# jmschrei/PyPore

Measured on AMD Instinct MI355X. Metric: Msamples/sec segmented (SpeedyStatSplit, 10^8-sample trace); %HBM roofline, higher is better.
Workload: dtype int32/f64 (exact integer block sums of fp32 or int16 samples; decisions in fp64)

## Files before the change

pypore_amd/csrc/poreseg.hip:

```cpp
#include <hip/hip_runtime.h>

#include <algorithm>
#include <atomic>
#include <chrono>
#include <complex>
#include <cmath>
#include <cstdarg>
#include <cstdio>
#include <cstdlib>
#include <cstring>
#include <initializer_list>
#include <condition_variable>
#include <mutex>
#include <string>
#include <thread>
#include <tuple>
#include <type_traits>
#include <vector>

#include "poreseg.h"
#include "seg_device.hpp"
#include "seg_align.hpp"
#include "seg_pairwise.hpp"
#include "seg_trf.hpp"
// ... 42 lines not shown
struct HostBuf : NoCopy {
    void *p = nullptr;
    size_t cap = 0;
    ~HostBuf() { release(); }
    hipError_t reserve(size_t bytes)
    {
        if (bytes <= cap) return hipSuccess;
        release();
        size_t want = std::max(bytes, cap + cap / 2);
        hipError_t e = hipHostMalloc(&p, want, hipHostMallocDefault);
        if (e == hipSuccess) { cap = want; g_live_bytes += cap; }
        return e;
    }
    void release() { if (p) { (void)hipHostFree(p); g_live_bytes -= cap; } p = nullptr; cap = 0; }
    template <class T> T *as() { return static_cast<T *>(p); }
};

struct Event : NoCopy {
    hipEvent_t e = nullptr;
    ~Event() { if (e) (void)hipEventDestroy(e); }
    operator hipEvent_t() const { return e; }
};

struct Stream : NoCopy {
    hipStream_t s = nullptr;
    bool own = false;
    ~Stream() { if (own && s) (void)hipStreamDestroy(s); }
    operator hipStream_t() const { return s; }
};

}

enum : int { SC_NO_LA = 1, SC_NO_UPLOAD = 2, SC_ALL = 3 };
constexpr int LA_KEEP = 16;
struct ps_ctx {
    int device = 0;
    int n_cu = 0;
    Stream stream;
    Event ev[10];
    Event ev_front[2];
    ~ps_ctx() { (void)hipSetDevice(device); if (stream.s) (void)hipStreamSynchronize(stream.s); }
    std::string err;
    int64_t tile_len = 0, halo = 0;
    int mode = MODE_FAST, spine_nt = 512, tree_nt = 256;
    int lds_max_samples = 0;
    int rep_eval = 1, rep_stage = 1, rep_sum = 1;
    uint8_t *d_is_spine = nullptr;
    int prune = 1;
    double wide_quantum = 0;
    int wide_skip = 0;
    int wide_mode = 0;
    int tree_mw = 0;
    int upload_by_kernel = 1;
    int k0_waves = 0;
    float noise_k = 0.1f;
    int k0_admit = 0;
    int k0_sets = 2;
    bool chain_held = false;
    unsigned long long chain_ticket = 0;
    bool defer_sync = false;
    int scan_lds_pad = 0;
    int k0_unaligned = 1;
    int single_pass = 1;
    int gather_fused = 1;
    int download_by_kernel = 1;
    int debug = 0;
// ... 37 lines not shown
    } trf;
    DevBuf ev_info_tr;
    DevBuf blk_cls, cls_mm;
    DevBuf pre_c;
    struct { DevBuf tab, pre, tmp, stack, cnt, off; } ss;
    struct { DevBuf tab, tab2, mask, cnt, excl, off1, off2, hits, pair_off, keep, kept, y, len, span_off; } sp;
    struct {
        DevBuf log;
        int64_t cap = 65536, hdr_cap = -1;
        int64_t seen = -1, call_cap = 0;
        std::vector<int64_t> ev_start, ev_len;
    } nt;
    struct {
        DevBuf model, off, bp, last, flags;
        std::vector<char> blob;
        long long bp_budget = 512ll << 20;
        DevBuf fmat, acc, skip;
        DevBuf pmax;
        DevBuf samp;
        long long fb_budget = 4ll << 30;
        bool expect_lds = true;
    } hmm;
    int stitch_host = 0;
    DevBuf ev_len, det_counts, det_tics, det_cand;
    DevBuf bridges, bmeta, tile_i32, sp_off, spine_items, asm_hdr, ev_first_tile;
    DevBuf bridge_ext, ext_slot, ext_list;
    DevBuf lat_state, lat_seam, lat_res;
    unsigned lat_tag_next = 1;
    unsigned lat_tag_base = 0;
    int lat_help = 1;
    int bridge_budget = BR_MAX;
    int bridge_ext_on = 1;
    int short_chain = SC_ALL;
    int shared_n = 0;
    int hw_queues = 0;
    int pool_patience = BR_PATIENCE_POOL;
    int la_keep = 0;
    bool la_now = false;
    bool small_clean = false;
    bool small_clean_in = false;
    HostBuf h_hdr;
    DevBuf spine_jobs, spine_scratch, spine_dense, spine_meta, tree_jobs, tree_scratch, tree_spill, tree_defer, screen_acc,
        tree_counts, items, item_pos, first_item, ev_off, bounds_off, small;
    HostBuf h_meta, h_dense, h_small, h_up;
    int timing = 1;
    double ms[8] = {0, 0, 0, 0, 0, 0, 0, 0};
    int64_t counters[20] = {0, 0, 0, 0, 0, 0, 0, 0, 0, 0, 0, 0, 0, 0, -1, -1, 0, 0, 0, 0};
    bool screen_ran = false;
};

namespace {

int fail(ps_ctx *ctx, int code, const char *fmt, ...)
{
    if (ctx) {
        char buf[512];
        va_list ap;
        va_start(ap, fmt);
        vsnprintf(buf, sizeof buf, fmt, ap);
        va_end(ap);
        ctx->err = buf;
    }
    return code;
}

#define HIP_TRY(ctx, expr)                                                                        \
// ... 73 lines not shown
    }
    c.left[t % K0Chain::RING] = t + 1;
    c.open_max = std::max(c.open_max, ++c.open);
    return PS_OK;
}
int chain_publish(ps_ctx *ctx, int device, hipStream_t st, unsigned long long ticket)
{
    K0Chain &c = g_chain[device & 15];
    std::lock_guard<std::mutex> lk(c.mu);
    const hipError_t e = hipEventRecord(c.ev[ticket % K0Chain::RING], st);
    c.close(ticket, e == hipSuccess);
    if (e != hipSuccess) return fail(ctx, PS_ERR_HIP, "hipEventRecord (K0 gate) failed: %s", hipGetErrorString(e));
    return PS_OK;
}
void chain_drop(ps_ctx *ctx)
{
    if (!ctx->chain_held) return;
    ctx->chain_held = false;
    K0Chain &c = g_chain[ctx->device & 15];
    std::lock_guard<std::mutex> lk(c.mu);
    c.close(ctx->chain_ticket, false);
}
constexpr size_t SMALL_TAIL = 64 * 1024;
struct SmallLayout { unsigned long long status, work0, work1, work2, dense, stamp[12], life[9], qctl, qhead, tree_tail; AsmHeader hdr;
                     unsigned long long lat_ctl[6]; int lat_prog[LAT_D];
                     unsigned long long nt_cur;
                     unsigned long long tree_defer[3]; };

int make_cfg(ps_ctx *ctx, const void *d_samples, const ps_sample_format *fmt, int mw, int maxw, int W,
             double min_gain, DevCfg *c)
{
    ctx->small_clean_in = ctx->small_clean;
    ctx->small_clean = false;
    if (!fmt) return fail(ctx, PS_ERR_ARG, "sample format is NULL");
    if (fmt->dtype != PS_DTYPE_F32 && fmt->dtype != PS_DTYPE_I16)
        return fail(ctx, PS_ERR_ARG, "unknown dtype %d", fmt->dtype);
    if (!(fmt->quantum > 0) || !std::isfinite(fmt->quantum))
        return fail(ctx, PS_ERR_ARG, "quantum must be positive and finite");
    c->samples = d_samples;
    c->dtype = fmt->dtype;
    c->off_counts = fmt->dtype == PS_DTYPE_F32 ? 0 : fmt->offset_counts;
    c->dc_counts = fmt->dtype == PS_DTYPE_F32 ? static_cast<double>(fmt->offset_counts) : 0.0;
    c->noise_k = ctx->noise_k;
    c->inv_q = static_cast<float>(1.0 / fmt->quantum);
    c->q = fmt->quantum;
    c->q2 = fmt->quantum * fmt->quantum;
    c->mw = mw; c->maxw = maxw; c->W = W; c->half = W / 2;
    c->min_gain = min_gain;
    c->mode = ctx->mode;
    c->prune = ctx->prune;
    c->lds_cap = std::max(1, std::min(W, ctx->lds_max_samples));
    c->bsum = nullptr; c->ev_info = nullptr; c->chunk_tot = nullptr; c->blk_mm = nullptr; c->grp = nullptr; c->bs_wide = 0;
    c->blk_cls = nullptr; c->cls_mm = nullptr; c->cls_kthr = 0;
    c->k0_unaligned = ctx->k0_unaligned;
    c->pre_c = nullptr; c->pre_c2 = nullptr;
    c->dbg = ctx->small.as<SmallLayout>()->stamp;
    c->nt_log = nullptr;
    c->rep_eval = ctx->rep_eval; c->rep_stage = ctx->rep_stage; c->rep_sum = ctx->rep_sum;
    return PS_OK;
}

inline size_t lds_bytes_for(int lds_cap, int nt)
{
    return (((static_cast<size_t>(lds_cap) + 32) * sizeof(lds_t) + 15) & ~static_cast<size_t>(15)) +
           (static_cast<size_t>(lds_cap) / PBLK + static_cast<size_t>(nt) + 8) * sizeof(int2);
}
// ... 243 lines not shown

inline int64_t spine_cap(int64_t start, int64_t stop, int mw) { return (stop - start) / mw + 4; }

struct TilePlace { int64_t first_tile = 0, ntiles = 1, tile_len = 0x7fffffff, vbase = 0; };
SpineJob make_spine_job(int64_t base, int32_t ev, int64_t len, int64_t start, int64_t stop, int mw, int64_t out_off,
                        const TilePlace &place = TilePlace())
{
    SpineJob j;
    j.base = base;
    j.start = static_cast<int32_t>(start);
    j.end = static_cast<int32_t>(len);
    j.stop = static_cast<int32_t>(stop);
    j.out_cap = static_cast<int32_t>(std::min<int64_t>(spine_cap(start, stop, mw), 0x7fffffff));
    j.out_off = out_off;
    j.first_tile = static_cast<int32_t>(place.first_tile);
    j.ntiles = static_cast<int32_t>(place.ntiles);
    j.tile_len = static_cast<int32_t>(place.tile_len);
    j.ev = ev;
    j.vbase = place.vbase;
    return j;
}

int find_in(const TileList &t, int32_t pos)
{
    if (pos == t.start) return -1;
    auto it = std::lower_bound(t.a.begin(), t.a.end(), pos, [](const Anchor &x, int32_t v) { return x.pos < v; });
    if (it != t.a.end() && it->pos == pos) return static_cast<int>(it - t.a.begin());
    return -2;
}

}

namespace {
constexpr int RC_FALLBACK = 1;
constexpr int RC_WIDE = 2;
int finish_batch(ps_ctx *ctx, const DevCfg &cfg, size_t n_tj, int64_t n_items, int32_t n_ev,
                        int32_t *d_bounds, int64_t cap, int64_t *h_bounds_off, ps_segstat *d_stats,
                        std::chrono::steady_clock::time_point t_begin, const AsmHeader *d_hdr = nullptr,
                        AsmHeader *hdr_out = nullptr, bool wide_check = false)
{
    int rc;
    const size_t evb = (static_cast<size_t>(n_ev) + 1) * sizeof(int64_t);
    SmallLayout *sm = ctx->small.as<SmallLayout>();
    if (ctx->timing >= 2) HIP_TRY(ctx, hipEventRecord(ctx->ev[2], ctx->stream));
    if (n_tj) {
        const unsigned g = static_cast<unsigned>(std::min<size_t>(n_tj, 0x7fffffff));
        if (int lrc = launch_subtrees(ctx, cfg, g, sm, n_tj, d_hdr)) return lrc;
    }
    if (ctx->timing >= 2) HIP_TRY(ctx, hipEventRecord(ctx->ev[3], ctx->stream));
    const bool fused = d_hdr != nullptr && ctx->gather_fused;
    const bool one_copy = ctx->bounds_off.p == ctx->small.as<char>() + sizeof(SmallLayout);
    int dl_clear = 0;
    if (fused) {
        const int64_t blocks = (n_items >> GS_LOG) + 1;
        const unsigned gg = static_cast<unsigned>(std::max<int64_t>(1, std::min<int64_t>(blocks, 1024)));
        hipLaunchKernelGGL(gather_scan_kernel, dim3(gg), dim3(1 << GS_LOG), 0, ctx->stream, ctx->items.as<Item>(),
                           ctx->tree_jobs.as<TreeJob>(), ctx->tree_counts.as<int32_t>(), ctx->tree_scratch.as<int32_t>(),
                           static_cast<long long>(n_items), d_bounds, cap, ctx->d_is_spine, d_hdr, ctx->first_item.as<int64_t>(),
                           n_ev, ctx->bounds_off.as<int64_t>());
        HIP_TRY(ctx, hipGetLastError());
    } else {
    hipLaunchKernelGGL(item_scan_kernel, dim3(1), dim3(1024), 0, ctx->stream, ctx->items.as<Item>(),
                       ctx->tree_counts.as<int32_t>(), n_items, ctx->item_pos.as<int64_t>(), d_hdr,
                       ctx->first_item.as<int64_t>(), n_ev, ctx->bounds_off.as<int64_t>());
    HIP_TRY(ctx, hipGetLastError());
    }
    if (n_items && !fused) {
        const unsigned gg = static_cast<unsigned>(d_hdr ? std::min<int64_t>(n_items, 16384) : n_items);
        hipLaunchKernelGGL(gather_kernel, dim3(gg), dim3(64), 0, ctx->stream,
                           ctx->items.as<Item>(), ctx->tree_jobs.as<TreeJob>(), ctx->tree_counts.as<int32_t>(),
                           ctx->tree_scratch.as<int32_t>(), ctx->item_pos.as<int64_t>(), n_items, d_bounds, cap, ctx->d_is_spine,
                           d_hdr);
        HIP_TRY(ctx, hipGetLastError());
    }
    const bool stats_from_digest = d_stats != nullptr && cfg.bsum != nullptr && cfg.blk_mm != nullptr;
    if (stats_from_digest) {
        const int64_t scap = cap + n_ev;
        const unsigned sg = static_cast<unsigned>(std::min<int64_t>(std::max<int64_t>(scap, 1), 8192));
        by_dtype(cfg.dtype, [&](auto dt) {
            hipLaunchKernelGGL(segstat_bs_kernel<dt()>, dim3(sg), dim3(64), 0, ctx->stream, cfg, ctx->ev_off.as<int64_t>(),
                               ctx->ev_len.as<int64_t>(), n_ev, d_bounds, ctx->bounds_off.as<int64_t>(), d_stats, scap,
                               reinterpret_cast<unsigned *>(&sm->status), d_hdr);
        });
        HIP_TRY(ctx, hipGetLastError());
        if (ctx->timing >= 2) HIP_TRY(ctx, hipEventRecord(ctx->ev[4], ctx->stream));
    }
    if (one_copy) {
        HIP_TRY(ctx, ctx->h_small.reserve(sizeof(SmallLayout) + evb));
// ... 446 lines not shown
#ifdef PS_DIAG
    if (ctx->dbg_phase == 2) {
        if (front) front_lock.unlock();
        HIP_TRY(ctx, hipStreamSynchronize(fs));
        for (int e = 0; e <= n_ev; ++e) h_bounds_off[e] = 0;
        return PS_OK;
    }
#endif
    if (front) {
        HIP_TRY(ctx, hipEventRecord(ctx->ev_front[1], fs));
        front_lock.unlock();
        HIP_TRY(ctx, hipStreamWaitEvent(ctx->stream, ctx->ev_front[1], 0));
    }
    if (nj) {
        const unsigned g = static_cast<unsigned>(nj);
        int lrc;
        if (wide) lrc = launch_scans_bs<DT_WIDE>(ctx, cfg, g, sm);
        else if (use_bs) lrc = launch_scans_bs<0>(ctx, cfg, g, sm);
        else {
            lrc = launch_spine_nt(ctx, cfg, g, sm, true);
            if (lrc) return lrc;
            if (ctx->timing >= 2) HIP_TRY(ctx, hipEventRecord(ctx->ev[6], ctx->stream));
            lrc = by_nt<256, 512>(ctx->spine_nt, [&](auto nt) {
                return by_dtype(cfg.dtype, [&](auto dt) { return launch_bridge<decltype(nt)::value, dt()>(ctx, cfg, g, sm); });
            });
        }
        if (lrc) return lrc;
    }
    if (ctx->timing >= 2) HIP_TRY(ctx, hipEventRecord(ctx->ev[1], ctx->stream));
    int *ti = ctx->tile_i32.as<int>();
    const size_t njp = std::max<size_t>(1, nj);
    const size_t tile_lds = (nj + 1) * sizeof(long long) + 4 * nj * sizeof(int);
    const int use_lds = tile_lds <= 150 * 1024;
    if (use_lds)
        HIP_TRY(ctx, set_dyn_lds(ctx, reinterpret_cast<const void *>(assemble_tiles_kernel), static_cast<int>(tile_lds)));
    AsmHeader hd = {};
    int rc = PS_OK;
    int64_t items_cap = max_items;
    int slots_used = 0, ext_stride = EXT_MAX;
    const bool no_la = nj && no_look_ahead(ctx, cfg);
    bool la_done = false, stride_set = false;
    for (int round = 0;; ++round) {
        hipLaunchKernelGGL(assemble_tiles_kernel, dim3(1), dim3(1024), use_lds ? tile_lds : 0, ctx->stream,
                           static_cast<int>(nj), ctx->spine_meta.as<int4>(), ctx->bmeta.as<int4>(),
                           ctx->ev_first_tile.as<int64_t>(), n_ev, ti, ti + njp, ti + 2 * njp, ti + 3 * njp,
                           ctx->sp_off.as<long long>(), ctx->first_item.as<int64_t>(), ctx->asm_hdr.as<AsmHeader>(),
                           static_cast<long long>(items_cap), use_lds, reinterpret_cast<const unsigned *>(&sm->status));
        HIP_TRY(ctx, hipGetLastError());
        const AsmHeader *d_hdr = ctx->asm_hdr.as<AsmHeader>();
        if (items_cap > 0) {
            const unsigned ag = static_cast<unsigned>(std::min<int64_t>((items_cap + 255) / 256, 2048));
            hipLaunchKernelGGL(assemble_items_kernel, dim3(ag), dim3(256), 0,
                               ctx->stream, ctx->spine_jobs.as<SpineJob>(), static_cast<int>(nj), ctx->spine_meta.as<int4>(),
                               ctx->spine_scratch.as<int2>(), ctx->bridges.as<int2>(), ti + 3 * njp,
                               ctx->sp_off.as<long long>(), static_cast<long long>(items_cap), mw, W, ctx->tree_jobs.as<TreeJob>(),
                               ctx->items.as<Item>(), ctx->tree_counts.as<int32_t>(), d_hdr, cfg.bsum != nullptr ? cfg.ev_info : nullptr,
                               ctx->bridge_ext.as<int2>(), ctx->ext_slot.as<int>(), ext_stride);
            HIP_TRY(ctx, hipGetLastError());
        }
        if (ctx->timing >= 2 && round == 0) HIP_TRY(ctx, hipEventRecord(ctx->ev[5], ctx->stream));
        rc = finish_batch(ctx, cfg, static_cast<size_t>(items_cap), items_cap, n_ev, d_bounds, cap, h_bounds_off, d_stats, t_begin,
                          d_hdr, &hd, use_bs);
        if (rc != RC_FALLBACK || !use_bs || !nj || round == EXT_ROUNDS + (la_done ? 1 : 0) || !ctx->bridge_ext_on) break;
        HIP_TRY(ctx, ctx->h_meta.reserve(2 * nj * sizeof(int4)));
        int4 *h_bm = ctx->h_meta.as<int4>(), *h_mt = h_bm + nj;
        HIP_TRY(ctx, hipMemcpyAsync(h_bm, ctx->bmeta.p, nj * sizeof(int4), hipMemcpyDeviceToHost, ctx->stream));
        HIP_TRY(ctx, hipMemcpyAsync(h_mt, ctx->spine_meta.p, nj * sizeof(int4), hipMemcpyDeviceToHost, ctx->stream));
        HIP_TRY(ctx, hipStreamSynchronize(ctx->stream));
        if (no_la && !la_done) {
            int64_t n_def = 0;
            for (size_t g = 0; g < nj; ++g) n_def += h_bm[g].w == BR_DEFER || h_bm[g].w == BR_DEFER_REACHED;
            if (n_def) {
                if (ctx->debug) fprintf(stderr, "[poreseg] look-ahead kernel behind the stitch: %lld deferred seams\n", static_cast<long long>(n_def));
                HIP_TRY(ctx, hipMemsetAsync(&sm->hdr, 0, sizeof(AsmHeader), ctx->stream));
                if (ctx->tree_screen) HIP_TRY(ctx, hipMemsetAsync(&sm->tree_defer[0], 0, sizeof sm->tree_defer[0], ctx->stream));
                if (int lrc = by_dtype(cfg.dtype, [&](auto dt) { return launch_bridge_la<dt()>(ctx, cfg, static_cast<unsigned>(nj), sm); })) return lrc;
                la_done = true;
                ctx->la_keep = LA_KEEP;
                ctx->counters[4] += n_def;
                ctx->counters[18] += n_def;
                continue;
            }
        }
        std::vector<int> list;
        bool hopeless = false;
        if (!stride_set) {
            size_t n_fail = 0;
            for (size_t g = 0; g < nj; ++g) n_fail += h_bm[g].w == BR_FAIL_REACHED || (h_bm[g].w == BR_FAIL && h_bm[g].x == ctx->bridge_budget);
            ext_stride = n_fail <= static_cast<size_t>(EXT_SLOTS) ? EXT_MAX : EXT_MAX_MANY;
            stride_set = true;
        }
        const int slot_cap = EXT_SLOTS * (EXT_MAX / ext_stride);
        for (size_t g = 0; g < nj; ++g) {
            const bool reached = h_bm[g].w == BR_FAIL_REACHED;
            const bool gave_up = h_bm[g].x == ctx->bridge_budget;
// ... 3 lines not shown
            if (slots_used + static_cast<int>(list.size()) < slot_cap) list.push_back(static_cast<int>(g));
            else if (reached) hopeless = true;
        }
        if (list.empty() || hopeless) break;
        if (ctx->debug) fprintf(stderr, "[poreseg] second chance, round %d: %zu seams continued on the device\n", round + 1, list.size());
        const size_t n_ext = list.size();
        HIP_TRY(ctx, ctx->bridge_ext.reserve(static_cast<size_t>(EXT_SLOTS) * EXT_MAX * sizeof(int2)));
        HIP_TRY(ctx, ctx->ext_slot.reserve(nj * sizeof(int)));
        HIP_TRY(ctx, ctx->ext_list.reserve(static_cast<size_t>(EXT_SLOTS) * (EXT_MAX / EXT_MAX_MANY) * sizeof(int)));
        HIP_TRY(ctx, hipMemcpyAsync(ctx->ext_list.p, list.data(), n_ext * sizeof(int), hipMemcpyHostToDevice, ctx->stream));
        HIP_TRY(ctx, hipStreamSynchronize(ctx->stream));
        HIP_TRY(ctx, hipMemsetAsync(&sm->hdr, 0, sizeof(AsmHeader), ctx->stream));
        if (ctx->tree_screen) HIP_TRY(ctx, hipMemsetAsync(&sm->tree_defer[0], 0, sizeof sm->tree_defer[0], ctx->stream));
        {
            const unsigned g = static_cast<unsigned>(n_ext);
            auto extend = [&](auto dt) {
                hipLaunchKernelGGL((bridge_la_kernel<dt(), true>), dim3(g), dim3(64 * BR_LA), 0, ctx->stream, cfg,
                                   ctx->spine_jobs.as<SpineJob>(), ctx->spine_scratch.as<int2>(), ctx->spine_meta.as<int4>(),
                                   ctx->bridges.as<int2>(), ctx->bmeta.as<int4>(), reinterpret_cast<unsigned *>(&sm->status),
                                   &sm->work0, static_cast<int>(n_ext), ctx->ext_list.as<int>(), ctx->bridge_ext.as<int2>(),
                                   ctx->ext_slot.as<int>(), slots_used, BR_MAX, ext_stride);
            };
            if (wide) by_dtype<DT_WIDE>(cfg.dtype, extend);
            else by_dtype(cfg.dtype, extend);
            HIP_TRY(ctx, hipGetLastError());
        }
        ctx->counters[4] += static_cast<int64_t>(n_ext);
        slots_used += static_cast<int>(n_ext);
        items_cap += static_cast<int64_t>(n_ext) * ext_stride;
        if (int irc = reserve_items(ctx, items_cap, total_len, mw)) return irc;
    }
    ctx->counters[3] = hd.n_items;
    if (slots_used > 0 || la_done) ctx->small_clean = false;
    float ms = 0;
    if (ctx->timing >= 2 && nj && hipEventElapsedTime(&ms, ctx->ev[7], ctx->ev[0]) == hipSuccess) ctx->ms[6] = ms;
    if (ctx->timing >= 2 && nj && hipEventElapsedTime(&ms, ctx->ev[0], ctx->ev[6]) == hipSuccess) ctx->ms[0] = ms;
    if (ctx->timing >= 2 && nj && hipEventElapsedTime(&ms, ctx->ev[6], ctx->ev[1]) == hipSuccess) ctx->ms[5] = ms;
    if (ctx->timing >= 2 && hipEventElapsedTime(&ms, ctx->ev[1], ctx->ev[5]) == hipSuccess) ctx->ms[4] = ms;
    return rc;
}
int device_stitch_batch(ps_ctx *ctx, const DevCfg &cfg_in, int bs_mode, const int64_t *ev_start, const int64_t *ev_len, int32_t n_ev, int mw, int W,
                        int32_t *d_bounds, int64_t cap, int64_t *h_bounds_off, ps_segstat *d_stats,
                        std::chrono::steady_clock::time_point t_begin, bool digest_ready = false)
{
    const int rc = device_stitch_batch_(ctx, cfg_in, bs_mode, ev_start, ev_len, n_ev, mw, W, d_bounds, cap, h_bounds_off, d_stats, t_begin, digest_ready);
    chain_drop(ctx);
    return rc;
}
}

namespace {
std::mutex g_probe_mu;
int g_unaligned_ok[16] = {-1, -1, -1, -1, -1, -1, -1, -1, -1, -1, -1, -1, -1, -1, -1, -1};
int k0_unaligned_probe(int device, hipStream_t st)
{
    std::lock_guard<std::mutex> lk(g_probe_mu);
    int &ok = g_unaligned_ok[device & 15];
    if (ok >= 0) return ok;
    ok = 0;
    unsigned char h[128];
    for (int i = 0; i < 128; ++i) h[i] = static_cast<unsigned char>(37 * i + 11);
    DevBuf d_buf, bad_buf;
    if (d_buf.reserve(256) != hipSuccess || bad_buf.reserve(sizeof(unsigned)) != hipSuccess) { (void)hipGetLastError(); return ok; }
    unsigned char *d = d_buf.as<unsigned char>();
    unsigned *bad = bad_buf.as<unsigned>();
    unsigned hb = 1;
// ... 157 lines not shown
    else if (n == "groups") ctx->groups = value != 0;
    else if (n == "tree_par") ctx->tree_par = value != 0;
    else if (n == "k0_waves" && value >= 0 && value <= 16) ctx->k0_waves = static_cast<int>(value);
    else if (n == "k0_shared") ctx->k0_shared = value != 0;
    else if (n == "k0_admit" && value >= 0) ctx->k0_admit = static_cast<int>(value);
    else if (n == "bridge_ext" && (value == 0 || value == 1)) ctx->bridge_ext_on = static_cast<int>(value);
    else if (n == "lat_help" && value >= 0 && value <= 2) ctx->lat_help = static_cast<int>(value);
    else if (n == "shared_device" && value >= 0 && value <= 4096) {
        ps_pool_plan_t plan;
        if (pool_plan(static_cast<int>(value), ctx->hw_queues > 0 ? ctx->hw_queues : process_hw_queues(), &plan) != PS_OK)
            return fail(ctx, PS_ERR_ARG, "shared_device: no plan for %lld contexts", static_cast<long long>(value));
        ctx->shared_n = static_cast<int>(value);
        ctx->la_keep = 0;
        ctx->k0_waves = plan.k0_waves;
        ctx->lat_help = plan.lat_help;
        ctx->k0_admit = plan.k0_admit;
    }
    else if (n == "hw_queues" && value >= 0 && value <= HW_QUEUES_MAX) ctx->hw_queues = static_cast<int>(value);
    else if (n == "hmm_bp_budget" && value >= 1) ctx->hmm.bp_budget = value;
    else if (n == "hmm_fb_budget" && value >= 1) ctx->hmm.fb_budget = value;
    else if (n == "pairwise_budget" && value >= 1) ctx->pw.budget = value;
    else if (n == "trf_budget" && value >= 1) ctx->trf.budget = value;
    else if (n == "hmm_expect_lds") ctx->hmm.expect_lds = value != 0;
    else if (n == "single_pass") ctx->single_pass = value != 0;
    else if (n == "gather_fused") ctx->gather_fused = value != 0;
    else if (n == "download_by_kernel") ctx->download_by_kernel = value != 0;
    else if (n == "debug") ctx->debug = value != 0;
    else if (n == "k0_unaligned") ctx->k0_unaligned = value != 0 ? k0_unaligned_probe(ctx->device, ctx->stream) : 0;
    else if (n == "slots_pct" && value >= 1 && value <= 100) ctx->slots_pct = static_cast<int>(value);
    else if (n == "tree_jobs_per_wave" && value >= 0 && value <= 1024) ctx->tree_jobs_per_wave = static_cast<int>(value);
    else if (n == "tree_screen") ctx->tree_screen = value != 0;
    else if (n == "short_chain" && value >= 0 && value <= 3) {
        static const int bits[4] = {0, SC_ALL, SC_NO_LA, SC_NO_UPLOAD};
        if (ctx->short_chain != bits[value]) ctx->small_clean = false;
        ctx->short_chain = bits[value];
    }
    else if (n == "bridge_patience" && value >= 1 && value <= 4096) { ctx->pool_patience = static_cast<int>(value); ctx->la_keep = 0; }
    else if (n == "noise_k_ppm" && value >= 0) ctx->noise_k = static_cast<float>(static_cast<double>(value) * 1.0e-6);
#ifdef PS_DIAG
    else if (n == "dbg_phase" && value >= 0 && value <= 2) ctx->dbg_phase = static_cast<int>(value);
    else if (n == "dbg_k0_nogrp") ctx->dbg_k0_nogrp = value != 0;
    else if (n == "cu_mask" && ctx->stream.own)
        return diag_mask_stream(ctx, &ctx->stream.s, static_cast<int>(value & 0xfff), static_cast<int>((value >> 12) & 0xfff),
                                static_cast<int>((value >> 24) & 0xff), ((value >> 32) & 1) != 0);
    else if (n == "k0_sets" && value >= 2 && value <= 4) ctx->k0_sets = static_cast<int>(value);
    else if (n == "scan_lds_pad" && value >= 0 && value <= 65536) ctx->scan_lds_pad = static_cast<int>(value);
    else if (n == "rep_eval" && value >= 1) ctx->rep_eval = static_cast<int>(value);
    else if (n == "rep_stage" && value >= 1) ctx->rep_stage = static_cast<int>(value);
    else if (n == "rep_sum" && value >= 1) ctx->rep_sum = static_cast<int>(value);
#endif
    else if (n == "bridge_budget" && value >= 1 && value <= BR_MAX) ctx->bridge_budget = static_cast<int>(value);
    else if (n == "wide_bs") { ctx->wide_bs = value != 0; ctx->wide_skip = 0; }
    else if (n == "bridge_single" && value >= 1) ctx->bridge_single = static_cast<int>(value);
    else if (n == "tree_tail_pct" && value >= 0 && value <= 100) ctx->tree_tail_pct = static_cast<int>(value);
    else if (n == "filter_fused") ctx->filt.fused = value != 0;
    else if (n == "upload_by_kernel") ctx->upload_by_kernel = value != 0;
    else if (n == "timing") ctx->timing = static_cast<int>(std::max<int64_t>(0, std::min<int64_t>(2, value)));
    else if (n == "tree_mw") ctx->tree_mw = value != 0;
    else if (n == "spine_nt" && (value == 256 || value == 512 || value == 1024)) ctx->spine_nt = static_cast<int>(value);
    else if (n == "tree_nt" && (value == 256 || value == 512)) ctx->tree_nt = static_cast<int>(value);
    else return fail(ctx, PS_ERR_ARG, "unknown option or value: %s", name);
    return PS_OK;
}

int ps_get_option(const ps_ctx *ctx, const char *name, int64_t *value)
{
    if (!ctx || !name || !value) return PS_ERR_ARG;
    const std::string n(name);
    if (n == "k0_waves") *value = ctx->k0_waves;
    else if (n == "k0_admit") *value = ctx->k0_admit;
    else if (n == "lat_help") *value = ctx->lat_help;
    else if (n == "shared_device") *value = ctx->shared_n;
    else if (n == "hw_queues") *value = ctx->hw_queues;
    else return PS_ERR_ARG;
    return PS_OK;
}

int ps_pool_plan(int32_t n_contexts, int32_t hw_queues, ps_pool_plan_t *out) { return pool_plan(n_contexts, hw_queues, out); }

int ps_hw_queues(void) { return process_hw_queues(); }

int ps_gate_stats(int device, int64_t *out, int32_t n_out, int reset)
{
    if (device < 0 || device >= 16 || (!out && n_out > 0) || n_out < 0) return PS_ERR_ARG;
    K0Chain &c = g_chain[device];
    std::lock_guard<std::mutex> lk(c.mu);
    const int64_t v[5] = {static_cast<int64_t>(c.next), c.open, c.open_max, c.host_waits, c.gave_up};
    for (int i = 0; i < n_out; ++i) out[i] = i < 5 ? v[i] : 0;
    if (reset) { c.open_max = c.open; c.host_waits = 0; c.gave_up = 0; }
    return PS_OK;
}

int ps_synchronize(ps_ctx *ctx)
{
    if (!ctx) return PS_ERR_ARG;
    HIP_TRY(ctx, hipStreamSynchronize(ctx->stream));
    return PS_OK;
}

int ps_min_gain(const ps_split_params *p, double *out)
{
    if (!p || !out) return PS_ERR_ARG;
    double fpr = p->false_positive_rate, sps = p->prior_segments_per_second;
    const double sf = p->sampling_freq;
    if (!(fpr != 0.0)) fpr = sf;
    if (!(sps != 0.0)) sps = sf / 2.;
// ... 2207 lines not shown
```

pypore_amd/csrc/seg_device.hpp:

```cpp
#pragma once
#include <hip/hip_runtime.h>
#include <stdint.h>
#include "poreseg.h"

namespace ps {

constexpr int LDS_STACK = 128;
constexpr int MAX_WAVES = 16;
constexpr int OBUF = 256;
constexpr int BR_MAX = 256;
constexpr int LST_MAX = 256;
constexpr int LAT_D = 256;
constexpr int LAT_W = 16;
constexpr int LAT_C = 2048;
constexpr int LAT_TAGS = 4096;
struct LatHelp {
    unsigned long long *ctl;
    unsigned long long *state;
    int *seam;
    int *prog;
    unsigned long long *res;
    unsigned tag_base;
    int stay;
};
// ... 2084 lines not shown
            if (b.w == BR_DEFER) bmeta[g].w = BR_DEFER_REACHED;
        }
    }
    __syncthreads();
    for (int g0 = 0; g0 < n_tiles; g0 += 1024) {
        const int g = g0 + tid;
        long long n = 0;
        if (g < n_tiles && reach[g]) {
            const int c = meta[g].x - entry[g];
            n = static_cast<long long>(c) + bmeta[g].x;
            if (c < 0) fail_s = 1;
        }
        long long e1, e2;
        chunk_exscan2(n, 0, e1, e2, wsum, carry);
        if (g < n_tiles) sp_off[g] = e1;
    }
    const long long n_items = carry[0];
    if (tid == 0) sp_off[n_tiles] = n_items;
    __syncthreads();
    for (int e = tid; e <= n_ev; e += 1024) first_item[e] = sp_off[ev_first_tile[e]];
    if (use_lds)
        for (int g = tid; g <= n_tiles; g += 1024) {
            sp_off_out[g] = sp_off[g];
            if (g < n_tiles) entry_out[g] = entry[g];
        }
    if (tid == 0) {
        hdr->n_items = n_items;
        hdr->n_jobs = n_items;
        hdr->tscratch = 0;
        hdr->fail = (fail_s || n_items > max_items) ? 1 : 0;
    }
}

__global__ __launch_bounds__(256) void assemble_items_kernel(
    const SpineJob *jobs, int n_tiles, const int4 *meta, const int2 *lists, const int2 *bridges,
    const int *entry, const long long *sp_off, long long n_items_host, int mw, int W,
    TreeJob *tjobs, Item *items, int32_t *counts, const AsmHeader *hdr, const int4 *ev_info,
    const int2 *ext = nullptr, const int *ext_slot = nullptr, int ext_stride = EXT_MAX)
{
    const long long n_items = dev_count(hdr, n_items_host);
    for (long long b = blockIdx.x * 256LL + threadIdx.x; b <= (n_items >> GS_LOG); b += gridDim.x * 256LL) counts[n_items_host + b] = 0;
    for (long long i = blockIdx.x * 256LL + threadIdx.x; i < n_items; i += gridDim.x * 256LL) {
    int lo = 0, hi = n_tiles - 1;
    while (lo < hi) {
        const int mid = (lo + hi) >> 1;
        if (sp_off[mid + 1] > i) hi = mid; else lo = mid + 1;
    }
    const int g = lo;
    const int k = static_cast<int>(i - sp_off[g]);
    const int en = entry[g], cnt = meta[g].x;
    const SpineJob jb2 = jobs[g];
    int2 el;
    int pred;
    if (k < cnt - en) {
        el = lists[jb2.out_off + en + k];
        pred = (en + k) > 0 ? lists[jb2.out_off + en + k - 1].x : jb2.start;
    } else {
        const int kb = k - (cnt - en);
        el = bridge_at(bridges, ext, ext_slot, ext_stride, g, kb);
        pred = kb > 0 ? bridge_at(bridges, ext, ext_slot, ext_stride, g, kb - 1).x : (cnt > 0 ? lists[jb2.out_off + cnt - 1].x : jb2.start);
    }
    const bool has = el.y == KIND_HIT || el.y == KIND_LATE;
    Item it;
    it.anchor = el.x;
    it.job = has ? static_cast<int32_t>(i) : -1;
    items[i] = it;
// ... 330 lines not shown
```

pypore_amd/engine.py:

```python
import collections
import ctypes
import os
import threading
import warnings

import numpy as np
import torch

from . import _lib

_contexts = {}

DEFAULT_OPTIONS = {}
DEFAULT_TILING = [0, 0]
POOL_OVERRIDES = {}

EVENT_CAP = 1 << 16

_ENV_OPTIONS = {
    "PORESEG_MODE": "mode", "PORESEG_SPINE_NT": "spine_nt", "PORESEG_TREE_NT": "tree_nt", "PORESEG_PRUNE": "prune",
    "PORESEG_SCAN_BS": "scan_bs", "PORESEG_GROUPS": "groups", "PORESEG_TREE_PAR": "tree_par", "PORESEG_K0_WAVES": "k0_waves",
    "PORESEG_K0_SHARED": "k0_shared", "PORESEG_K0_MAX": "k0_admit", "PORESEG_K0_SETS": "k0_sets", "PORESEG_WIDE_BS": "wide_bs",
    "PORESEG_BRIDGE_SINGLE": "bridge_single", "PORESEG_TREE_TAIL": "tree_tail_pct", "PORESEG_FILTER_FUSED": "filter_fused",
    "PORESEG_UPLOAD": "upload_by_kernel", "PORESEG_TIMING": "timing", "PORESEG_TREE_MW": "tree_mw",
    "PORESEG_TREE_JPW": "tree_jobs_per_wave", "PORESEG_TREE_SCREEN": "tree_screen", "PORESEG_SLOTS_PCT": "slots_pct", "PORESEG_BRIDGE_EXT": "bridge_ext",
    "PORESEG_LAT_HELP": "lat_help", "PORESEG_BRIDGE_BUDGET": "bridge_budget", "PORESEG_DEBUG": "debug",
    "PORESEG_SHORT_CHAIN": "short_chain", "PORESEG_BRIDGE_PATIENCE": "bridge_patience",
    "PORESEG_GATHER_FUSED": "gather_fused", "PORESEG_SINGLE_PASS": "single_pass", "PORESEG_DOWNLOAD": "download_by_kernel", "PORESEG_K0_UNALIGNED": "k0_unaligned",
    "PORESEG_DBG_PHASE": "dbg_phase", "PORESEG_DBG_K0_NOGRP": "dbg_k0_nogrp", "PORESEG_SCAN_LDS_PAD": "scan_lds_pad", "PORESEG_REP_STAGE": "rep_stage",
}


def options_from_env(environ=None):
    env = os.environ if environ is None else environ
    opts = {}
    for var, name in _ENV_OPTIONS.items():
        if var in env and env[var] != "":
            opts[name] = int(env[var])
    if env.get("PORESEG_STITCH"):
        opts["stitch_host"] = 1 if env["PORESEG_STITCH"] == "host" else 0
    if "PORESEG_NOISE_K" in env:
        opts["noise_k_ppm"] = int(round(float(env["PORESEG_NOISE_K"]) * 1e6))
    tiling = [int(env.get("PORESEG_TILE", "0") or 0), int(env.get("PORESEG_HALO", "0") or 0)]
    pool = {}
    if "PORESEG_POOL_K0_WAVES" in env:
        pool["k0_waves"] = int(env["PORESEG_POOL_K0_WAVES"])
    if "PORESEG_POOL_K0_MAX" in env:
        pool["k0_admit"] = int(env["PORESEG_POOL_K0_MAX"])
    if env.get("PORESEG_POOL_SHARED", "0") == "1":
        pool["k0_shared"] = 1
    return opts, tiling, pool


def apply_env_defaults(environ=None):
    opts, tiling, pool = options_from_env(environ)
    DEFAULT_OPTIONS.update(opts)
    if tiling[0] or tiling[1]:
        DEFAULT_TILING[:] = tiling
    POOL_OVERRIDES.update(pool)
    return opts, tiling, pool
# ... 57 lines not shown
            pass

    def set_tiling(self, tile_len=0, halo=0):
        with self.lock:
            _lib.check(self.L.ps_set_tiling(self.handle, int(tile_len), int(halo)), self.handle)

    def set_option(self, name, value):
        with self.lock:
            _lib.check(self.L.ps_set_option(self.handle, name.encode(), int(value)), self.handle)

    def get_option(self, name):
        out = ctypes.c_int64()
        self.L.ps_get_option.argtypes = [ctypes.c_void_p, ctypes.c_char_p, ctypes.POINTER(ctypes.c_int64)]
        with self.lock:
            _lib.check(self.L.ps_get_option(self.handle, name.encode(), ctypes.byref(out)), self.handle)
        return int(out.value)

    def seq_ms(self):
        if not hasattr(self, "_tm"):
            self._tm = ((ctypes.c_double * 8)(), (ctypes.c_int64 * 8)())
        self.L.ps_get_timings(self.handle, self._tm[0], 8, self._tm[1], 8)
        return self._tm[0][7]

    def timings(self):
        ms = (ctypes.c_double * 8)()
        cnt = (ctypes.c_int64 * 20)()
        _lib.check(self.L.ps_get_timings(self.handle, ms, 8, cnt, 20))
        return dict(spine_ms=ms[0], tree_ms=ms[1], gather_ms=ms[2], total_ms=ms[3], stitch_ms=ms[4], bridge_ms=ms[5], blocksum_ms=ms[6], seq_ms=ms[7],
                    windows=cnt[0], candidates=cnt[1], tiles=cnt[2], tree_jobs=cnt[3], repairs=cnt[4],
                    exact_rescans=cnt[5], full_exact_scans=cnt[6], wide_redo=cnt[7],
                    windows_spine=cnt[8], windows_bridge=cnt[9], windows_tree=cnt[10], near_ties=cnt[11],
                    helper_chunks_published=cnt[12], helper_chunks_taken=cnt[13],
                    tree_deferred=cnt[14], windows_screen=cnt[15],
                    lookahead_skipped=cnt[16], upload_skipped=cnt[17], seams_resumed=cnt[18])

    def near_ties(self):
        if not hasattr(self, "_cnt"):
            self._cnt = self.L.ps_counters(self.handle)
        return int(self._cnt[11])

    def near_tie_sites(self):
        with self.lock:
            n = ctypes.c_int64()
            cap = 64
            while True:
                buf = (_lib.NearTie * cap)()
                rc = self.L.ps_get_near_ties(self.handle, buf, cap, ctypes.byref(n))
                if rc == _lib.PS_ERR_CAPACITY and n.value > cap:
                    cap = int(n.value)
                    continue
                _lib.check(rc, self.handle)
                break
            if n.value < 0:
                return None
            return np.frombuffer(buf, dtype=NEAR_TIE_DTYPE, count=int(n.value)).copy()

    @_serialised
    def segment_batch(self, samples, ev_off, params, quantum, offset_counts=0, want_stats=True, cap=None,
                      want_spine=False, lead=0, out=None, near_tie_warning=True):
        assert samples.is_cuda and samples.is_contiguous() and samples.dim() == 1
        if samples.dtype == torch.float32:
            dtype = _lib.PS_DTYPE_F32
        elif samples.dtype == torch.int16:
            dtype = _lib.PS_DTYPE_I16
        else:
            raise ValueError("samples must be float32 or int16, got %s" % samples.dtype)
        ev_off = np.ascontiguousarray(ev_off, dtype=np.int64)
# ... 952 lines not shown
```

Measured before the change: 604,400.

## Add lean single-block tile assembly and size item grids from previous call

```diff
diff --git a/pypore_amd/csrc/poreseg.hip b/pypore_amd/csrc/poreseg.hip
--- a/pypore_amd/csrc/poreseg.hip
+++ b/pypore_amd/csrc/poreseg.hip
@@ -98,6 +98,7 @@
 }
 
 enum : int { SC_NO_LA = 1, SC_NO_UPLOAD = 2, SC_ALL = 3 };
+enum : int { LL_TILES = 1, LL_GRIDS = 2, LL_ALL = 3 };
 constexpr int LA_KEEP = 16;
 struct ps_ctx {
     int device = 0;
@@ -201,6 +202,9 @@
     int bridge_budget = BR_MAX;
     int bridge_ext_on = 1;
     int short_chain = SC_ALL;
+    int lean_launch = LL_ALL;
+    int64_t prev_items = -1;
+    int64_t prev_items_in = -1;
     int shared_n = 0;
     int hw_queues = 0;
     int pool_patience = BR_PATIENCE_POOL;
@@ -340,6 +344,8 @@
 {
     ctx->small_clean_in = ctx->small_clean;
     ctx->small_clean = false;
+    ctx->prev_items_in = ctx->prev_items;
+    ctx->prev_items = -1;
     if (!fmt) return fail(ctx, PS_ERR_ARG, "sample format is NULL");
     if (fmt->dtype != PS_DTYPE_F32 && fmt->dtype != PS_DTYPE_I16)
         return fail(ctx, PS_ERR_ARG, "unknown dtype %d", fmt->dtype);
@@ -649,12 +655,16 @@
 }
 
 namespace {
+unsigned lean_grid(int64_t items)
+{
+    return static_cast<unsigned>(std::min<int64_t>(std::max<int64_t>(64, (2 * items + 255) / 256 + 1), 0x7fffffff));
+}
 constexpr int RC_FALLBACK = 1;
 constexpr int RC_WIDE = 2;
 int finish_batch(ps_ctx *ctx, const DevCfg &cfg, size_t n_tj, int64_t n_items, int32_t n_ev,
                         int32_t *d_bounds, int64_t cap, int64_t *h_bounds_off, ps_segstat *d_stats,
                         std::chrono::steady_clock::time_point t_begin, const AsmHeader *d_hdr = nullptr,
-                        AsmHeader *hdr_out = nullptr, bool wide_check = false)
+                        AsmHeader *hdr_out = nullptr, bool wide_check = false, int64_t lean_items = -1)
 {
     int rc;
     const size_t evb = (static_cast<size_t>(n_ev) + 1) * sizeof(int64_t);
@@ -670,7 +680,8 @@
     int dl_clear = 0;
     if (fused) {
         const int64_t blocks = (n_items >> GS_LOG) + 1;
-        const unsigned gg = static_cast<unsigned>(std::max<int64_t>(1, std::min<int64_t>(blocks, 1024)));
+        unsigned gg = static_cast<unsigned>(std::max<int64_t>(1, std::min<int64_t>(blocks, 1024)));
+        if (lean_items >= 0) gg = std::min(gg, lean_grid(lean_items));
         hipLaunchKernelGGL(gather_scan_kernel, dim3(gg), dim3(1 << GS_LOG), 0, ctx->stream, ctx->items.as<Item>(),
                            ctx->tree_jobs.as<TreeJob>(), ctx->tree_counts.as<int32_t>(), ctx->tree_scratch.as<int32_t>(),
                            static_cast<long long>(n_items), d_bounds, cap, ctx->d_is_spine, d_hdr, ctx->first_item.as<int64_t>(),
@@ -1183,7 +1194,12 @@
     const size_t njp = std::max<size_t>(1, nj);
     const size_t tile_lds = (nj + 1) * sizeof(long long) + 4 * nj * sizeof(int);
     const int use_lds = tile_lds <= 150 * 1024;
-    if (use_lds)
+    const bool lean_rt = nj && short_route(ctx, cfg);
+    const bool lean_tiles = lean_rt && (ctx->lean_launch & LL_TILES) && nj <= static_cast<size_t>(TL_CAP);
+    int64_t lean_items = lean_rt && (ctx->lean_launch & LL_GRIDS) && reuse ? ctx->prev_items_in : -1;
+    ctx->prev_items_in = -1;
+    ctx->counters[19] = (lean_tiles ? LL_TILES : 0) | (lean_items >= 0 ? LL_GRIDS : 0);
+    if (use_lds && !lean_tiles)
         HIP_TRY(ctx, set_dyn_lds(ctx, reinterpret_cast<const void *>(assemble_tiles_kernel), static_cast<int>(tile_lds)));
     AsmHeader hd = {};
     int rc = PS_OK;
@@ -1192,6 +1208,14 @@
     const bool no_la = nj && no_look_ahead(ctx, cfg);
     bool la_done = false, stride_set = false;
     for (int round = 0;; ++round) {
+        if (round > 0) lean_items = -1;
+        if (lean_tiles)
+            hipLaunchKernelGGL(assemble_tiles_lean_kernel, dim3(1), dim3(TL_NT), 0, ctx->stream,
+                               static_cast<int>(nj), ctx->spine_meta.as<int4>(), ctx->bmeta.as<int4>(),
+                               ctx->ev_first_tile.as<int64_t>(), n_ev, ti + 3 * njp, ctx->sp_off.as<long long>(),
+                               ctx->first_item.as<int64_t>(), ctx->asm_hdr.as<AsmHeader>(), static_cast<long long>(items_cap),
+                               reinterpret_cast<const unsigned *>(&sm->status));
+        else
         hipLaunchKernelGGL(assemble_tiles_kernel, dim3(1), dim3(1024), use_lds ? tile_lds : 0, ctx->stream,
                            static_cast<int>(nj), ctx->spine_meta.as<int4>(), ctx->bmeta.as<int4>(),
                            ctx->ev_first_tile.as<int64_t>(), n_ev, ti, ti + njp, ti + 2 * njp, ti + 3 * njp,
@@ -1200,7 +1224,8 @@
         HIP_TRY(ctx, hipGetLastError());
         const AsmHeader *d_hdr = ctx->asm_hdr.as<AsmHeader>();
         if (items_cap > 0) {
-            const unsigned ag = static_cast<unsigned>(std::min<int64_t>((items_cap + 255) / 256, 2048));
+            unsigned ag = static_cast<unsigned>(std::min<int64_t>((items_cap + 255) / 256, 2048));
+            if (lean_items >= 0) ag = std::min(ag, lean_grid(lean_items));
             hipLaunchKernelGGL(assemble_items_kernel, dim3(ag), dim3(256), 0,
                                ctx->stream, ctx->spine_jobs.as<SpineJob>(), static_cast<int>(nj), ctx->spine_meta.as<int4>(),
                                ctx->spine_scratch.as<int2>(), ctx->bridges.as<int2>(), ti + 3 * njp,
@@ -1211,7 +1236,7 @@
         }
         if (ctx->timing >= 2 && round == 0) HIP_TRY(ctx, hipEventRecord(ctx->ev[5], ctx->stream));
         rc = finish_batch(ctx, cfg, static_cast<size_t>(items_cap), items_cap, n_ev, d_bounds, cap, h_bounds_off, d_stats, t_begin,
-                          d_hdr, &hd, use_bs);
+                          d_hdr, &hd, use_bs, lean_items);
         if (rc != RC_FALLBACK || !use_bs || !nj || round == EXT_ROUNDS + (la_done ? 1 : 0) || !ctx->bridge_ext_on) break;
         HIP_TRY(ctx, ctx->h_meta.reserve(2 * nj * sizeof(int4)));
         int4 *h_bm = ctx->h_meta.as<int4>(), *h_mt = h_bm + nj;
@@ -1281,6 +1306,7 @@
     }
     ctx->counters[3] = hd.n_items;
     if (slots_used > 0 || la_done) ctx->small_clean = false;
+    ctx->prev_items = (rc == PS_OK && !hd.fail && slots_used == 0 && !la_done) ? static_cast<int64_t>(hd.n_items) : -1;
     float ms = 0;
     if (ctx->timing >= 2 && nj && hipEventElapsedTime(&ms, ctx->ev[7], ctx->ev[0]) == hipSuccess) ctx->ms[6] = ms;
     if (ctx->timing >= 2 && nj && hipEventElapsedTime(&ms, ctx->ev[0], ctx->ev[6]) == hipSuccess) ctx->ms[0] = ms;
@@ -1504,8 +1530,13 @@
     else if (n == "tree_screen") ctx->tree_screen = value != 0;
     else if (n == "short_chain" && value >= 0 && value <= 3) {
         static const int bits[4] = {0, SC_ALL, SC_NO_LA, SC_NO_UPLOAD};
-        if (ctx->short_chain != bits[value]) ctx->small_clean = false;
+        if (ctx->short_chain != bits[value]) { ctx->small_clean = false; ctx->prev_items = -1; }
         ctx->short_chain = bits[value];
+    }
+    else if (n == "lean_launch" && value >= 0 && value <= 3) {
+        static const int bits[4] = {0, LL_ALL, LL_TILES, LL_GRIDS};
+        if (ctx->lean_launch != bits[value]) ctx->prev_items = -1;
+        ctx->lean_launch = bits[value];
     }
     else if (n == "bridge_patience" && value >= 1 && value <= 4096) { ctx->pool_patience = static_cast<int>(value); ctx->la_keep = 0; }
     else if (n == "noise_k_ppm" && value >= 0) ctx->noise_k = static_cast<float>(static_cast<double>(value) * 1.0e-6);
@@ -1544,6 +1575,7 @@
     else if (n == "lat_help") *value = ctx->lat_help;
     else if (n == "shared_device") *value = ctx->shared_n;
     else if (n == "hw_queues") *value = ctx->hw_queues;
+    else if (n == "lean_launch") { static const int values[4] = {0, 2, 3, 1}; *value = values[ctx->lean_launch & 3]; }
     else return PS_ERR_ARG;
     return PS_OK;
 }
diff --git a/pypore_amd/csrc/seg_device.hpp b/pypore_amd/csrc/seg_device.hpp
--- a/pypore_amd/csrc/seg_device.hpp
+++ b/pypore_amd/csrc/seg_device.hpp
@@ -2140,6 +2140,166 @@
     }
 }
 
+#ifndef PS_TL_NT
+#define PS_TL_NT 1024
+#endif
+constexpr int TL_NT = PS_TL_NT;
+constexpr int TL_CAP = 4096;
+constexpr int TL_PER = TL_CAP / TL_NT;
+constexpr unsigned short TL_NONE = 0xffffu;
+static_assert(TL_CAP <= TL_NONE, "tile indices and the sentinel share 16 bits");
+
+__global__ __launch_bounds__(TL_NT) void assemble_tiles_lean_kernel(
+    int n_tiles, const int4 *meta, int4 *bmeta, const int64_t *ev_first_tile, int n_ev, int *entry_out, long long *sp_off,
+    int64_t *first_item, AsmHeader *hdr, long long max_items, const unsigned *status)
+{
+    __shared__ unsigned short tab[TL_CAP];
+    __shared__ unsigned reach[TL_CAP / 32];
+    __shared__ long long wtot[TL_PER][TL_NT / 64];
+    __shared__ int fail_s;
+    const int tid = threadIdx.x, lane = tid & 63, wave = tid >> 6;
+    const bool fits = n_tiles <= TL_CAP;
+    const unsigned st = *status;
+    int4 bm[TL_PER];
+    int mx[TL_PER];
+#pragma unroll
+    for (int k = 0; k < TL_PER; ++k) {
+        const int g = tid + k * TL_NT;
+        bm[k] = make_int4(0, 0, 0, BR_NONE);
+        mx[k] = 0;
+        if (fits && g < n_tiles) { bm[k] = bmeta[g]; mx[k] = meta[g].x; }
+    }
+    int64_t t0 = 0, t1 = 0;
+    if (tid < n_ev) { t0 = ev_first_tile[tid]; t1 = ev_first_tile[tid + 1]; }
+    if ((st & ST_WIDE_RANGE) != 0u || !fits) {
+        if (tid == 0) { hdr->n_items = 0; hdr->n_jobs = 0; hdr->tscratch = 0; hdr->fail = 1; hdr->pad = 0; }
+        return;
+    }
+    auto reached = [&](int g) { return (reach[g >> 5] >> (g & 31)) & 1u; };
+    auto joined = [&](const int4 &b) { return b.w == BR_JOINED && static_cast<unsigned>(b.y) < static_cast<unsigned>(n_tiles); };
+    const int n_chunks = (n_tiles + TL_NT - 1) / TL_NT;
+    if (tid == 0) fail_s = 0;
+    for (int w = tid; w < TL_CAP / 32; w += TL_NT) reach[w] = 0u;
+#pragma unroll
+    for (int k = 0; k < TL_PER; ++k) {
+        const int g = tid + k * TL_NT;
+        if (g < n_tiles) tab[g] = joined(bm[k]) ? static_cast<unsigned short>(bm[k].y) : TL_NONE;
+    }
+    __syncthreads();
+    if (tid < n_ev && t0 < t1) atomicOr(&reach[t0 >> 5], 1u << (t0 & 31));
+    for (int e = tid + TL_NT; e < n_ev; e += TL_NT) {
+        const int64_t f = ev_first_tile[e];
+        if (f < ev_first_tile[e + 1]) atomicOr(&reach[f >> 5], 1u << (f & 31));
+    }
+    __syncthreads();
+    int rounds = 1;
+    while ((1 << rounds) < n_tiles) ++rounds;
+    for (int r = 0; r <= rounds; ++r) {
+        unsigned short nxt[TL_PER];
+#pragma unroll
+        for (int k = 0; k < TL_PER; ++k) {
+            const int g = tid + k * TL_NT;
+            nxt[k] = TL_NONE;
+            if (k < n_chunks && g < n_tiles) {
+                const unsigned short j = tab[g];
+                if (j != TL_NONE) {
+                    if (reached(g)) atomicOr(&reach[j >> 5], 1u << (j & 31));
+                    nxt[k] = tab[j];
+                }
+            }
+        }
+        __syncthreads();
+#pragma unroll
+        for (int k = 0; k < TL_PER; ++k) {
+            const int g = tid + k * TL_NT;
+            if (k < n_chunks && g < n_tiles) tab[g] = nxt[k];
+        }
+        __syncthreads();
+    }
+    unsigned mine = 0u;
+#pragma unroll
+    for (int k = 0; k < TL_PER; ++k) {
+        const int g = tid + k * TL_NT;
+        if (g < n_tiles) { if (reached(g)) mine |= 1u << k; tab[g] = 0; }
+    }
+    __syncthreads();
+#pragma unroll
+    for (int k = 0; k < TL_PER; ++k) {
+        if (!((mine >> k) & 1u)) continue;
+        const int g = tid + k * TL_NT;
+        const int4 b = bm[k];
+        if (joined(b)) {
+            const int v = b.z + 1;
+            if (v >= 0 && v < static_cast<int>(TL_NONE)) tab[b.y] = static_cast<unsigned short>(v);
+            else { tab[b.y] = TL_NONE; entry_out[b.y] = v; }
+        }
+        if (b.w == BR_FAIL || b.w == BR_DEFER || b.w == BR_FAIL_REACHED || b.w == BR_DEFER_REACHED) {
+            fail_s = 1;
+            if (b.w == BR_FAIL) bmeta[g].w = BR_FAIL_REACHED;
+            if (b.w == BR_DEFER) bmeta[g].w = BR_DEFER_REACHED;
+        }
+    }
+    __syncthreads();
+    long long excl[TL_PER];
+#pragma unroll
+    for (int k = 0; k < TL_PER; ++k) {
+        excl[k] = 0;
+        if (k >= n_chunks) continue;
+        const int g = tid + k * TL_NT;
+        long long n = 0;
+        if (g < n_tiles) {
+            int en = tab[g];
+            if (en == static_cast<int>(TL_NONE)) en = entry_out[g];
+            entry_out[g] = en;
+            if ((mine >> k) & 1u) {
+                const int c = mx[k] - en;
+                n = static_cast<long long>(c) + bm[k].x;
+                if (c < 0) fail_s = 1;
+            }
+        }
+        long long inc = n;
+#pragma unroll
+        for (int d = 1; d < 64; d <<= 1) {
+            const long long u = __shfl_up(inc, d);
+            if (lane >= d) inc += u;
+        }
+        if (lane == 63) wtot[k][wave] = inc;
+        excl[k] = inc - n;
+    }
+    __syncthreads();
+    long long run = 0;
+#pragma unroll
+    for (int k = 0; k < TL_PER; ++k) {
+        if (k >= n_chunks) continue;
+        long long base = run;
+#pragma unroll
+        for (int w = 0; w < TL_NT / 64; ++w) {
+            const long long v = wtot[k][w];
+            if (w < wave) base += v;
+            run += v;
+        }
+        const int g = tid + k * TL_NT;
+        if (g < n_tiles) sp_off[g] = base + excl[k];
+    }
+    const long long n_items = run;
+    if (tid == 0) sp_off[n_tiles] = n_items;
+    if (n_ev <= 1) {
+        if (tid <= n_ev) first_item[tid] = tid == 0 ? 0 : n_items;
+    } else {
+        __syncthreads();
+        for (int e = tid; e <= n_ev; e += TL_NT) {
+            const int64_t f = ev_first_tile[e];
+            first_item[e] = f <= 0 ? 0 : (f >= n_tiles ? n_items : sp_off[f]);
+        }
+    }
+    if (tid == 0) {
+        hdr->n_items = n_items;
+        hdr->n_jobs = n_items;
+        hdr->tscratch = 0;
+        hdr->fail = (fail_s || n_items > max_items) ? 1 : 0;
+    }
+}
+
 __global__ __launch_bounds__(256) void assemble_items_kernel(
     const SpineJob *jobs, int n_tiles, const int4 *meta, const int2 *lists, const int2 *bridges,
     const int *entry, const long long *sp_off, long long n_items_host, int mw, int W,
diff --git a/pypore_amd/engine.py b/pypore_amd/engine.py
--- a/pypore_amd/engine.py
+++ b/pypore_amd/engine.py
@@ -25,7 +25,7 @@
     "PORESEG_UPLOAD": "upload_by_kernel", "PORESEG_TIMING": "timing", "PORESEG_TREE_MW": "tree_mw",
     "PORESEG_TREE_JPW": "tree_jobs_per_wave", "PORESEG_TREE_SCREEN": "tree_screen", "PORESEG_SLOTS_PCT": "slots_pct", "PORESEG_BRIDGE_EXT": "bridge_ext",
     "PORESEG_LAT_HELP": "lat_help", "PORESEG_BRIDGE_BUDGET": "bridge_budget", "PORESEG_DEBUG": "debug",
-    "PORESEG_SHORT_CHAIN": "short_chain", "PORESEG_BRIDGE_PATIENCE": "bridge_patience",
+    "PORESEG_SHORT_CHAIN": "short_chain", "PORESEG_BRIDGE_PATIENCE": "bridge_patience", "PORESEG_LEAN_LAUNCH": "lean_launch",
     "PORESEG_GATHER_FUSED": "gather_fused", "PORESEG_SINGLE_PASS": "single_pass", "PORESEG_DOWNLOAD": "download_by_kernel", "PORESEG_K0_UNALIGNED": "k0_unaligned",
     "PORESEG_DBG_PHASE": "dbg_phase", "PORESEG_DBG_K0_NOGRP": "dbg_k0_nogrp", "PORESEG_SCAN_LDS_PAD": "scan_lds_pad", "PORESEG_REP_STAGE": "rep_stage",
 }
@@ -149,7 +149,8 @@
                     windows_spine=cnt[8], windows_bridge=cnt[9], windows_tree=cnt[10], near_ties=cnt[11],
                     helper_chunks_published=cnt[12], helper_chunks_taken=cnt[13],
                     tree_deferred=cnt[14], windows_screen=cnt[15],
-                    lookahead_skipped=cnt[16], upload_skipped=cnt[17], seams_resumed=cnt[18])
+                    lookahead_skipped=cnt[16], upload_skipped=cnt[17], seams_resumed=cnt[18],
+                    lean_launch=cnt[19])
 
     def near_ties(self):
         if not hasattr(self, "_cnt"):
```

After: 597,500. -1.1%, worse.
